# unum-cloud/usearch

Measured on AMD Instinct MI355X. Metric: QPS at recall@10>=0.95, 10000000x768 f16 cos, batch=10000, higher is better.
Workload: dtype f16

## Files before the change

usearch_amd/csrc/common.hpp:

```cpp
#pragma once
#include <cstddef>
#include <cstdint>

namespace usearch_amd {

enum metric_kind_t : std::uint8_t {
    metric_unknown_k = 0,
    metric_ip_k = 'i',
    metric_cos_k = 'c',
    metric_l2sq_k = 'e',
    metric_hamming_k = 'b',
    metric_pearson_k = 'p',
    metric_haversine_k = 'h',
    metric_divergence_k = 'd',
    metric_jaccard_k = 'j',
    metric_tanimoto_k = 't',
    metric_sorensen_k = 's',
};

enum scalar_kind_t : std::uint8_t {
    scalar_unknown_k = 0,
    scalar_b1x8_k = 1,
    scalar_bf16_k = 4,
    scalar_f64_k = 10,
// ... 46 lines not shown
    std::uint32_t dimensions;
    std::uint32_t m, m0;
    std::uint32_t max_level;
    std::uint32_t entry_slot;
    std::uint32_t has_tombstones;
    const std::uint8_t* sketch;
    const float* sketch_directions;
};

struct search_args_t {
    const std::uint8_t* queries;
    std::uint64_t query_stride;
    const std::uint32_t* todo;
    std::uint32_t count;
    std::uint32_t wanted;
    std::uint32_t ef;
    std::uint64_t* keys;
    float* distances;
    std::uint64_t* counts;
    std::uint64_t* visited;
    std::uint64_t* computed;
    std::uint32_t* status;
    std::uint32_t* queue;
    std::uint32_t* peaks;
    std::uint32_t hash_cap;
    std::uint32_t next_cap;
    std::uint8_t* scratch;
    std::uint64_t scratch_stride;
    const std::uint32_t* query_ids;
    std::uint32_t beam_level;
    std::uint32_t emit_slots;
    std::uint32_t descent_only;
    const std::uint32_t* allow_bits;
    const std::uint32_t* known_bits;
    std::uint32_t* ask_slots;
    std::uint64_t* ask_keys;
    std::uint32_t* ask_cursor;
    std::uint32_t ask_cap;
    std::uint32_t guess_threshold;
    std::uint32_t exclude_own;
    unsigned long long* phases;
    std::uint32_t team_offset;
    unsigned long long* wave_clock;
    std::uint32_t seen_offset;
    std::uint32_t seen_cells;
    std::uint32_t early_rows;
    std::uint32_t probe_mode;
    std::uint32_t claim_offset;
    std::uint32_t claim_bits;
    std::uint32_t aside_offset;
    std::uint32_t aside_cells;
    unsigned long long* sketch_counters;
    std::uint32_t sketch_offset;
};

enum : std::uint32_t { status_done_k = 0, status_overflow_k = 1 };

enum probe_mode_t : std::uint32_t {
    probe_swap_k = 0,
    probe_load_first_k = 1,
    probe_plain_k = 2,
};

}
```

usearch_amd/csrc/engine.hip:

```cpp
#include "engine.hpp"

#include <algorithm>
#include <atomic>
#include <chrono>
#include <cstdio>
#include <cstdlib>
#include <cstring>
#include <thread>

#include <hipcub/hipcub.hpp>

#include "casts.hpp"
#include "host_util.hpp"
#include "kernels.hpp"

namespace usearch_amd {

static constexpr std::uint32_t default_probe_mode_k = probe_swap_k;
static constexpr std::size_t default_early_rows_k = 1;

static hipError_t scratch_malloc(void** out, std::size_t bytes) {
#ifdef USEARCH_AMD_EXPERIMENT_SCRATCH_MEMORY
    const std::size_t kind = env_size("USEARCH_AMD_SCRATCH_MEMORY", 0);
    if (kind == 1 || kind == 2) {
// ... 674 lines not shown
        return "Unknown scratch mode";
    const bool top_in_memory = tuning.top_in_memory || env_size("USEARCH_AMD_TOP_IN_MEMORY", 0) != 0;
    const bool two_cells = lanes_ <= 2 && ef <= 128 && !env_size("USEARCH_AMD_NO_TWO_CELLS", 0);
    const std::uint32_t entries_per_lane = top_in_memory ? 0u : ef <= 64 ? 1u : two_cells ? 2u : ef <= 256 ? 4u : ef <= 512 ? 8u : ef <= 1024 ? 16u : 0u;
    call.entries_per_lane = entries_per_lane;

    const std::uint32_t frontier_request = tuning.frontier ? tuning.frontier : (std::uint32_t)env_size("USEARCH_AMD_FRONTIER", 0);
    const bool filtered = view_.has_tombstones || (extras && (extras->allow_bits || extras->exclude_own));
    const bool in_top_possible = frontier_in_top_capable(scalar_) && entries_per_lane && !filtered && mode_request != 3 &&
                                 view_.size < 0x80000000ull && !(extras && (extras->reference_frontier || extras->descent_only));
    if (frontier_request == 2 && !in_top_possible)
        return "The frontier cannot ride in `top` for this search (integer-valued pair, filter, tombstones or expansion > 1024)";
    const int frontier = (frontier_request == 1 || !in_top_possible) ? frontier_heap_k : frontier_top_k;
    if (frontier == frontier_top_k)
        next_cap = 0;

    const std::uint32_t chunks_per_lane = view_.chunks / lanes_;
    std::uint32_t variant_request = tuning.variant ? tuning.variant : (std::uint32_t)env_size("USEARCH_AMD_VARIANT", 0);
    int variant = variant_u4_w4_k;
    const bool every_build = lanes_ == 8 && all_kernel_builds(kernel_metric(metric_), scalar_);
    if (every_build && chunks_per_lane >= 8) {
        variant = chunks_per_lane >= 12 ? variant_u12_w2_k : variant_u8_w3_k;
        if (frontier == frontier_top_k && chunks_per_lane >= 12)
            variant = count >= 40000 ? variant_u4_w4_k : variant_u12x2_w2_k;
    }
    if (variant_request && variant_request - 1 < (std::uint32_t)variant_count_k && every_build) {
        const int requested = (int)variant_request - 1;
        if (requested == variant_u12x2_w2_k && frontier != frontier_top_k)
            return "That kernel build exists for the in-`top` frontier only";
        variant = requested;
    }
    const bool team = every_build && chunks_per_lane >= 8 && !variant_request && mode_request != 3 &&
                      count <= 2ull * compute_units_ && !(extras && extras->descent_only) && !env_size("USEARCH_AMD_NO_TEAM", 0) &&
                      !tuning.waves_per_cu;
    if (team)
        variant = variant_u12_w2_k;
    call.plain_possible = !team && !view_.has_tombstones && view_.m0 <= 64 && view_.nbr0 &&
                          !(extras && (extras->query_ids || extras->beam_level || extras->descent_only || extras->allow_bits || extras->exclude_own)) &&
                          (lanes_ == 1 ? view_.nbr0_rows != nullptr && view_.chunks == 1 : lanes_ == 2) &&
                          plain_build_exists(kernel_metric(metric_), scalar_, (int)lanes_, variant == variant_u4_w4_k, true, (int)entries_per_lane,
                                             frontier == frontier_heap_k) &&
                          !env_size("USEARCH_AMD_NO_PLAIN", 0);
    const std::uint32_t variant_waves_per_cu =
        4u * (std::uint32_t)kernel_waves(variant, (int)entries_per_lane, frontier, (int)lanes_, call.plain_possible);
    const std::uint32_t waves_cap = tuning.waves_per_cu ? tuning.waves_per_cu
                                                        : (std::uint32_t)env_size("USEARCH_AMD_WAVES_PER_CU", 32);
    call.waves_cap = std::min(waves_cap, variant_waves_per_cu);

    if (tuning.sketch > 2)
        return "Unknown sketch mode";
    const bool sketch_use = view_.sketch && tuning.sketch != 1 && !team && mode_request != 3 &&
                            (variant == variant_u12_w2_k || variant == variant_u12x2_w2_k) &&
                            !(extras && (extras->query_ids || extras->beam_level || extras->descent_only || extras->reference_frontier));
    const std::uint32_t sketch_lds = sketch_use ? sketch_columns_k * 4 + 16 : 0;
    auto lds_bytes_for = [&](int mode, std::uint32_t cap_next, std::uint32_t cap_hash) -> std::uint64_t {
        if (mode == scratch_global_k)
            return query_lds;
        const scratch_layout_t l = scratch_layout(entries_per_lane ? 0 : ef, cap_next,
                                                  mode == scratch_lds_k ? (std::uint64_t)cap_hash * 4 : 0);
        return query_lds + l.total + sketch_lds;
    };
    auto waves_for = [&](std::uint64_t lds_bytes) -> std::uint32_t {
        const std::uint64_t granule = (lds_bytes + lds_granule_k - 1) / lds_granule_k * lds_granule_k;
        return (std::uint32_t)std::max<std::uint64_t>(
            1, std::min<std::uint64_t>(call.waves_cap, lds_budget / std::max<std::uint64_t>(granule, 1)));
    };
    const bool default_next_cap = !tuning.next_cap && !env_size("USEARCH_AMD_NEXT_CAP", 0);
    if (default_next_cap && next_cap && mode_request != 1 && mode_request != 3) {
        const std::uint32_t now = waves_for(lds_bytes_for(scratch_hash_k, next_cap, hash_cap));
        if (now < call.waves_cap) {
            const std::uint64_t room = lds_budget / (now + 1) / lds_granule_k * lds_granule_k;
            const std::uint64_t fixed = lds_bytes_for(scratch_hash_k, 0, hash_cap);
            if (room > fixed) {
                const std::uint32_t trimmed = (std::uint32_t)((room - fixed) / 8 / 2 * 2);
                if (trimmed < next_cap && trimmed + 128 >= next_cap)
                    next_cap = trimmed;
            }
        }
    }
    std::uint64_t lds_mode_bytes = lds_bytes_for(scratch_lds_k, next_cap, hash_cap);
    if (!tuning.hash_cap && !env_size("USEARCH_AMD_HASH_CAP", 0) && mode_request == 0 && lds_mode_bytes > lds_budget) {
        const std::uint32_t tighter = std::min<std::uint32_t>(
            pow2_ceil(std::max<std::uint32_t>(1024, (ef * 30 + 1600) / 3 * 4)),
            pow2_ceil((std::uint32_t)std::min<std::uint64_t>(view_.size * 2 + 128, 1u << 30)));
        const std::uint64_t tighter_bytes = lds_bytes_for(scratch_lds_k, next_cap, tighter);
        if (tighter < hash_cap && tighter_bytes <= lds_budget && count <= (std::uint64_t)waves_for(tighter_bytes) * compute_units_ &&
            !env_size("USEARCH_AMD_NO_SMALL_BATCH_LDS", 0)) {
            hash_cap = tighter;
            lds_mode_bytes = tighter_bytes;
        }
    }
    const bool small_batch = lds_mode_bytes <= lds_budget && count <= (std::uint64_t)waves_for(lds_mode_bytes) * compute_units_ &&
                             !env_size("USEARCH_AMD_NO_SMALL_BATCH_LDS", 0);
    int mode = mode_request == 1 ? scratch_lds_k : mode_request == 2 ? scratch_hash_k : mode_request == 3 ? scratch_global_k
               : (small_batch || waves_for(lds_mode_bytes) >= std::min<std::uint32_t>(8, call.waves_cap) ? scratch_lds_k : scratch_hash_k);
    call.mode = mode;
    call.hash_cap = hash_cap;
    call.next_cap = next_cap;

    if (const char* e = ws.reserve(count, 0))
        return e;

    search_args_t& args = call.args;
    args = search_args_t{};
    args.queries = static_cast<const std::uint8_t*>(queries);
    args.query_stride = stride_bytes;
    args.wanted = (std::uint32_t)wanted;
// ... 134 lines not shown
            }
            args.aside_offset = 0, args.aside_cells = 0;
            const bool plain_wanted = call.plain_possible && !args.query_ids && !args.beam_level && !args.descent_only && !args.allow_bits &&
                                      !args.exclude_own && args.probe_mode == probe_swap_k && (lanes_ == 1 || args.early_rows != 0);
#ifdef USEARCH_AMD_EXPERIMENT_NO_ASIDE
            const bool aside_wanted = false;
#else
            const bool aside_wanted = plain_wanted && lanes_ == 2;
#endif
            if (aside_wanted) {
                std::uint32_t aside_cells = 512;
                if (const std::size_t forced_cells = env_size("USEARCH_AMD_ASIDE_CELLS", 0))
                    for (aside_cells = 64; aside_cells * 2 <= forced_cells && aside_cells < 2048; aside_cells *= 2) {}
                const std::uint64_t expected_visits = std::min<std::uint64_t>((std::uint64_t)call.ef * 20 + 800, view_.size);
                const bool room = expected_visits * expected_visits / (2ull * call.hash_cap) <= aside_cells * 3ull / 4 ||
                                  env_size("USEARCH_AMD_PLAIN_WHATEVER_THE_ROOM", 0);
                const std::uint64_t with_aside = (wave_lds_bytes + 15) / 16 * 16 + aside_cells * 4ull;
                if (room && waves_for(with_aside) >= waves_for(wave_lds_bytes) && with_aside <= lds_budget) {
                    args.aside_offset = (std::uint32_t)((wave_lds_bytes + 15) / 16 * 16);
                    args.aside_cells = aside_cells;
                    wave_lds_bytes = with_aside;
                }
            }
            const std::size_t forced = env_size("USEARCH_AMD_SEEN_CELLS", (std::size_t)-1);
            std::uint32_t cells = 0;
            if (forced != (std::size_t)-1) {
                for (cells = 1; cells * 2 <= forced && cells < 8192; cells *= 2) {}
                cells = forced ? cells : 0;
            } else {
                for (std::uint32_t candidate = 2048; candidate >= 128 && !cells; candidate /= 2)
                    if (waves_for((wave_lds_bytes + 15) / 16 * 16 + candidate * 4ull) >= waves_for(wave_lds_bytes))
                        cells = candidate;
            }
            if (cells && (wave_lds_bytes + 15) / 16 * 16 + cells * 4ull <= lds_budget) {
                args.seen_offset = (std::uint32_t)((wave_lds_bytes + 15) / 16 * 16);
                args.seen_cells = cells;
                wave_lds_bytes = args.seen_offset + cells * 4ull;
            }
            call.stats.probe_mode = args.probe_mode;
            call.stats.seen_cells = args.seen_cells;
            call.stats.claim_bits = args.claim_bits;
        }
        params.plain = 0;
        if (call.mode == scratch_hash_k && !params.team && lanes_ <= 2 && call.plain_possible && !args.query_ids && !args.beam_level &&
            !args.descent_only && !args.allow_bits && !args.exclude_own && args.probe_mode == probe_swap_k && (lanes_ == 1 || args.early_rows != 0)) {
#ifdef USEARCH_AMD_EXPERIMENT_NO_ASIDE
            params.plain = args.seen_cells ? 1u : 0u;
#else
            params.plain = (lanes_ == 2 ? args.aside_cells : args.seen_cells) ? 1u : 0u;
#endif
        }
        call.stats.plain = params.plain;
        call.stats.aside_cells = args.aside_cells;
        args.sketch_offset = 0;
        if (args.sketch_counters) {
            const std::uint64_t offset = (wave_lds_bytes + 15) / 16 * 16;
            if (!params.team && offset + sketch_columns_k * 4 <= lds_budget) {
                args.sketch_offset = (std::uint32_t)offset;
                wave_lds_bytes = offset + sketch_columns_k * 4;
            } else {
                args.sketch_counters = nullptr;
            }
        }
        const std::uint64_t lds_bytes = params.team ? (wave_lds_bytes + 15) / 16 * 16 + team_bytes : wave_lds_bytes;
        args.team_offset = params.team ? (std::uint32_t)((wave_lds_bytes + 15) / 16 * 16) : 0u;
        const std::uint32_t grid = params.team ? pending
                                               : (std::uint32_t)std::min<std::uint64_t>(pending, (std::uint64_t)waves_for(lds_bytes) * compute_units_);
        const std::uint64_t slab = call.mode == scratch_hash_k ? (std::uint64_t)call.hash_cap * 4 : 0;
        const std::size_t scratch_draws = std::min<std::size_t>(8, env_size("USEARCH_AMD_SCRATCH_DRAWS", 8));
        const bool draw_scratch = slab * grid > ws.scratch_bytes && slab * grid >= ((std::uint64_t)8 << 20) && scratch_draws > 1 &&
                                  pending >= 2ull * grid && grid >= 2u * (std::uint32_t)compute_units_ &&
                                  !env_size("USEARCH_AMD_SCRATCH_REDRAW", 0);
        if (const char* e = ws.reserve(call.count, draw_scratch ? 0 : slab * grid))
            return e;
        args.status = ws.d_status, args.peaks = ws.d_peaks;
        args.hash_cap = call.hash_cap;
        args.next_cap = call.next_cap;
        args.todo = call.have_todo ? ws.d_todo : nullptr;
        args.count = pending;
        args.scratch = ws.d_scratch;
        args.scratch_stride = slab;
        args.wave_clock = nullptr;
        if (draw_scratch) {
            params.mode = call.mode;
            params.entries_per_lane = call.entries_per_lane;
            params.grid = grid;
            params.lds_bytes = (std::uint32_t)lds_bytes;
            hipEvent_t begin = nullptr, end = nullptr;
            UA_HIP(hipEventCreate(&begin));
            if (hipError_t created = hipEventCreate(&end); created != hipSuccess) {
                (void)hipEventDestroy(begin);
                return hip_message(created);
            }
            void* candidates[8] = {nullptr};
            float trial_ms[8] = {0};
            std::size_t drawn = 0;
            const char* failure = nullptr;
            auto trial = [&](void* block, float& ms) -> const char* {
                args.scratch = static_cast<std::uint8_t*>(block);
                args.count = grid;
                for (int repeat = 0; repeat < 2; ++repeat) {
                    hipError_t e = hipMemsetAsync(ws.d_queue, 0, 8, stream);
                    if (e == hipSuccess)
                        e = hipEventRecord(begin, stream);
                    if (e == hipSuccess)
                        e = launch_search(metric_, scalar_, params, view_, args);
                    if (e == hipSuccess)
                        e = hipEventRecord(end, stream);
                    if (e == hipSuccess)
                        e = hipEventSynchronize(end);
                    if (e == hipSuccess)
                        e = hipEventElapsedTime(&ms, begin, end);
// ... 182 lines not shown
            std::memcpy(counters, ws.h_status + 2, 16);
            call.stats.sketch_tested += counters[0], call.stats.sketch_pruned += counters[1];
        }
        if (call.params.mode == scratch_global_k) {
            if (ws.h_status[1])
                return "Search scratch overflow in the global-memory pass";
            break;
        }
        if (!ws.h_status[1])
            break;
        UA_HIP(hipMemcpyAsync(ws.h_status + 16, ws.d_status, call.count * 4, hipMemcpyDeviceToHost, stream));
        UA_HIP(hipStreamSynchronize(stream));
        std::vector<std::uint32_t> again;
        if (call.have_todo) {
            for (std::uint32_t q : call.todo)
                if (ws.h_status[16 + q] == status_overflow_k)
                    again.push_back(q);
        } else {
            for (std::uint32_t q = 0; q < call.count; ++q)
                if (ws.h_status[16 + q] == status_overflow_k)
                    again.push_back(q);
        }
        call.todo.swap(again);
        call.have_todo = true;
        call.reran = true;
        if (call.todo.empty())
            break;
        if (rung == 0) {
            call.stats.retried_lds = (std::uint32_t)call.todo.size();
            call.mode = scratch_hash_k;
            call.hash_cap = std::min<std::uint32_t>(call.hash_cap * 4, pow2_ceil((std::uint32_t)std::min<std::uint64_t>(view_.size * 2 + 128, 1u << 30)));
            if (call.next_cap) {
                const std::uint32_t lds_budget = (std::uint32_t)env_size("USEARCH_AMD_LDS_BUDGET", 160 * 1024);
                call.next_cap = (std::uint32_t)std::min<std::uint64_t>((std::uint64_t)call.next_cap * 4, view_.size + 64);
                while (call.next_cap > 64 &&
                       call.query_lds + scratch_layout(call.entries_per_lane ? 0 : call.ef, call.next_cap, 0).total > lds_budget)
                    call.next_cap = call.next_cap * 3 / 4;
            }
        } else {
            call.mode = scratch_global_k;
        }
        if (call.mode != scratch_global_k)
            UA_HIP(hipMemcpyAsync(ws.d_todo, call.todo.data(), call.todo.size() * 4, hipMemcpyHostToDevice, stream));
        if (const char* e = run_ladder(call))
            return e;
    }

    if (call.want_phases) {
        unsigned long long ticks[16] = {0};
        UA_HIP(hipMemcpy(ticks, call.args.phases, 128, hipMemcpyDeviceToHost));
        double total = 0;
        for (int i = 0; i < 6; ++i)
            total += (double)ticks[i];
        std::fprintf(stderr, "[usearch_amd] phases ef=%u grid=%u: setup %.1f%% pop+list %.1f%% visited %.1f%% distances %.1f%% "
                             "commit %.1f%% [heap push %.1f%% top insert %.1f%%, %llu candidates rechecked] dump %.1f%% (%.3g ticks); "
                             "frontier pushes %llu, lists ready ahead %llu\n",
                     call.ef, first_grid, 100 * ticks[0] / total, 100 * ticks[1] / total, 100 * ticks[2] / total,
                     100 * ticks[3] / total, 100 * ticks[4] / total, 100 * ticks[8] / total, 100 * ticks[9] / total, ticks[10],
                     100 * ticks[5] / total, total, ticks[6], ticks[7]);
        if (ticks[15])
            std::fprintf(stderr, "[usearch_amd] a team's helpers: %llu hops, ticks measuring per hop %.0f %.0f %.0f %.0f\n", ticks[15],
                         (double)ticks[11] / (double)ticks[15], (double)ticks[12] / (double)ticks[15],
                         (double)ticks[13] / (double)ticks[15], (double)ticks[14] / (double)ticks[15]);
    }
    if (call.want_clock && ws.d_wave_clock && first_grid) {
        std::vector<unsigned long long> clock((std::size_t)first_grid * 2);
        UA_HIP(hipMemcpy(clock.data(), ws.d_wave_clock, clock.size() * 8, hipMemcpyDeviceToHost));
        unsigned long long first = ~0ull, last = 0;
        for (std::uint32_t w = 0; w < first_grid; ++w)
            first = std::min(first, clock[2 * w]), last = std::max(last, clock[2 * w + 1]);
        double gone = 0;
        for (std::uint32_t w = 0; w < first_grid; ++w)
            gone += (double)(clock[2 * w] - first) + (double)(last - clock[2 * w + 1]);
        const double span = (double)(last - first);
        call.stats.tail_idle = span > 0 ? (float)(gone / (span * first_grid)) : 0.f;
        call.stats.span_ms = (float)(span / 1e5);
        if (env_size("USEARCH_AMD_WAVE_CLOCK", 0) > 1) {
            unsigned long long bins[10] = {0};
            for (std::uint32_t w = 0; w < first_grid; ++w)
                ++bins[std::min<std::size_t>(9, (std::size_t)(10.0 * (double)(clock[2 * w + 1] - first) / std::max(span, 1.0)))];
            std::fprintf(stderr, "[usearch_amd] wave exits by tenth of the %.3f ms span (grid %u):", call.stats.span_ms, first_grid);
            for (unsigned long long b : bins)
                std::fprintf(stderr, " %llu", b);
            std::fprintf(stderr, "; idle share %.4f\n", call.stats.tail_idle);
        }
    }
    call.stats.passes = call.passes;
    call.stats.kernel_ms = call.total_ms;
    call.stats.mode = (std::uint32_t)first_mode + 1;
    call.stats.grid = first_grid;
    call.stats.lds_bytes = first_lds;
    if (stats)
        *stats = call.stats;
    if (call.sketch_auto && call.count >= 1024)
        judge_sketch(call.stats.sketch_tested, call.stats.sketch_pruned);
    return nullptr;
}

const char* snapshot_t::search_device(const void* queries, std::size_t count, std::size_t stride_bytes,
                                      std::size_t wanted, std::size_t expansion, std::uint64_t* keys,
                                      float* distances, std::uint64_t* counts, std::uint64_t* visited,
                                      std::uint64_t* computed, hipStream_t stream, const search_tuning_t& tuning,
                                      search_stats_t* stats, bool timed, const search_extras_t* extras) {
    if (stats)
        *stats = search_stats_t{};
    search_call_t call;
    const char* error = search_begin(call, queries, count, stride_bytes, wanted, expansion, keys, distances, counts, visited,
                                     computed, stream, tuning, timed, extras);
    if (error) {
        if (call.workspace)
            give_back(call.workspace);
        return error;
// ... 466 lines not shown
```

usearch_amd/csrc/kernels.hpp:

```cpp
#pragma once
#include <type_traits>
#include <hip/hip_runtime.h>

#include "common.hpp"
#include "sketch.hpp"

namespace usearch_amd {

#define UA_DEVICE __device__ __forceinline__


UA_DEVICE std::uint32_t lane_id() { return threadIdx.x & 63u; }

template <bool global_ak> UA_DEVICE void wave_sync() {
    if constexpr (global_ak) {
        __builtin_amdgcn_fence(__ATOMIC_RELEASE, "workgroup");
        __builtin_amdgcn_wave_barrier();
        __builtin_amdgcn_fence(__ATOMIC_ACQUIRE, "workgroup");
    } else {
        __builtin_amdgcn_fence(__ATOMIC_RELEASE, "workgroup", "local");
        __builtin_amdgcn_wave_barrier();
        __builtin_amdgcn_fence(__ATOMIC_ACQUIRE, "workgroup", "local");
    }
}
// ... 960 lines not shown
UA_DEVICE void team_touch_rows(const snapshot_view_t& ix, const std::uint32_t* ahead, std::uint32_t helper, team_landing_t& landing) {
    const std::uint32_t lane = lane_id();
    const std::uint32_t row = helper * 8 + (lane >> 3);
    const std::uint32_t slot = row < team_ahead_rows_k ? ahead[row] : none_slot_k;
    const std::uint32_t halves = (ix.bytes_per_vector + 63u) / 64u;
    const std::uint8_t* half = ix.vectors + (std::uint64_t)slot * ix.row_stride + (lane & 7u) * 64u;
    if (slot != none_slot_k && (lane & 7u) < halves)
        asm volatile("global_load_dword %0, %1, off" : "=&v"(landing.cell[0]) : "v"(half) : "memory");
    if (slot != none_slot_k && 8u + (lane & 7u) < halves)
        asm volatile("global_load_dword %0, %1, off" : "=&v"(landing.cell[1]) : "v"(half + 512) : "memory");
    if (slot != none_slot_k && 16u + (lane & 7u) < halves)
        asm volatile("global_load_dword %0, %1, off" : "=&v"(landing.cell[2]) : "v"(half + 1024) : "memory");
}
UA_DEVICE void team_landing_alive(const team_landing_t& landing) {
    asm volatile("" ::"v"(landing.cell[0]), "v"(landing.cell[1]), "v"(landing.cell[2]));
}

constexpr int team_waves_k = 5;

UA_DEVICE void team_barrier() { asm volatile("s_waitcnt lgkmcnt(0)\n\ts_barrier" ::: "memory"); }

template <int metric_ak, int scalar_ak, int lanes_ak, int loads_ak>
UA_DEVICE void team_share(const snapshot_view_t& ix, const std::uint8_t* query_lds, query_norm_t a2, const std::uint32_t* slots,
                          float* out, std::uint32_t count, std::uint32_t part, std::uint32_t parts, bool in_turn = false) {
    const std::uint32_t per_part = in_turn ? 64u / lanes_ak : (count + parts - 1) / parts;
    const std::uint32_t begin = part * per_part;
    const std::uint32_t end = (in_turn && part + 1 == parts) || begin + per_part > count ? count : begin + per_part;
    if (begin < end)
        measure_rows<metric_ak, scalar_ak, lanes_ak, loads_ak, false, 1>(ix, query_lds, a2, slots + begin, out + begin, end - begin);
}

template <int metric_ak, int scalar_ak, int lanes_ak, int unroll_ak, int mode_ak, int epl_ak, int frontier_ak, int team_ak = 1,
          bool plain_ak = false>
UA_DEVICE bool search_one(const snapshot_view_t& ix, const search_args_t& args, std::uint32_t q,
                          std::uint8_t* query_lds, std::uint8_t* heaps, std::uint32_t* visits, team_t* team = nullptr) {
    constexpr bool global_ak = mode_ak == scratch_global_k;
    constexpr bool in_top_ak = frontier_ak == frontier_top_k;
    static_assert(!in_top_ak || (epl_ak > 0 && !global_ak), "the frontier rides in the register layout of `top`");
    static_assert(!plain_ak || (lanes_ak <= 2 && mode_ak == scratch_hash_k && team_ak == 1 && !in_top_ak), "short rows over the global hash");
    using mem = scratch_gt<global_ak>;
    const std::uint32_t lane = lane_id();
    const std::uint32_t ef = args.ef, wanted = args.wanted;
    const scratch_layout_t layout = scratch_layout(epl_ak ? 0 : ef, in_top_ak ? 0 : args.next_cap, 0);
    top_gt<epl_ak, global_ak, in_top_ak> top;
    top.reset(reinterpret_cast<cand_t*>(heaps + layout.top));
    cand_t* next = reinterpret_cast<cand_t*>(heaps + layout.next);
    std::uint32_t* cand_slots = reinterpret_cast<std::uint32_t*>(heaps + layout.cand_slots);
    float* cand_distances = reinterpret_cast<float*>(heaps + layout.cand_distances);
    const std::uint32_t visits_mask = global_ak ? 0u : args.hash_cap - 1;
    const std::uint32_t visits_limit = global_ak ? 0xFFFFFFFFu : args.hash_cap - args.hash_cap / 4;

#ifdef USEARCH_AMD_PHASES
    std::uint64_t phase_mark = args.phases ? __builtin_amdgcn_s_memtime() : 0;
    std::uint64_t phase_ticks[6] = {0, 0, 0, 0, 0, 0};
    std::uint32_t diagnostic_pushes = 0, diagnostic_ready = 0, diagnostic_rechecks = 0;
    std::uint64_t diagnostic_push_ticks = 0, diagnostic_insert_ticks = 0;
    auto tick = [&](int phase) {
        if (args.phases) {
            const std::uint64_t now = __builtin_amdgcn_s_memtime();
            phase_ticks[phase] += now - phase_mark;
            phase_mark = now;
        }
    };
#else
    auto tick = [](int) {};
#endif
    const std::uint64_t query_row = !plain_ak && args.query_ids ? args.query_ids[q] : q;
    const query_norm_t a2 = stage_query<metric_ak, scalar_ak, lanes_ak>(
        ix, args.queries + query_row * args.query_stride, query_lds);

    if constexpr (!global_ak) {
        uint4* cells = reinterpret_cast<uint4*>(visits);
        const uint4 empty = {none_slot_k, none_slot_k, none_slot_k, none_slot_k};
        for (std::uint32_t i = lane; i < args.hash_cap / 4; i += 64)
            cells[i] = empty;
#ifdef USEARCH_AMD_EXPERIMENT_NO_SLAB_CLEAR_WAIT
        wave_sync<false>();
#else
        if constexpr (mode_ak == scratch_hash_k)
            wave_sync<true>();
        else
            wave_sync<false>();
#endif
    }

    constexpr bool seen_ak = lanes_ak <= 2 && mode_ak == scratch_hash_k && team_ak == 1;
#ifdef USEARCH_AMD_EXPERIMENT_NO_ASIDE
    constexpr bool aside_ak = false;
#else
    constexpr bool aside_ak = plain_ak && lanes_ak == 2;
#endif
    std::uint32_t* seen = nullptr;
    std::uint32_t seen_mask = 0;
    std::uint32_t* aside = nullptr;
    std::uint32_t aside_mask = 0, aside_count = 0;
    if constexpr (aside_ak) {
        aside = reinterpret_cast<std::uint32_t*>(query_lds + args.aside_offset);
        aside_mask = args.aside_cells - 1;
        for (std::uint32_t i = lane; i < args.aside_cells; i += 64)
            aside[i] = none_slot_k;
        wave_sync<false>();
    }
    if constexpr (seen_ak) {
        if (args.seen_cells) {
            seen = reinterpret_cast<std::uint32_t*>(query_lds + args.seen_offset);
            seen_mask = args.seen_cells - 1;
            for (std::uint32_t i = lane; i < args.seen_cells; i += 64)
// ... 38 lines not shown
        }
    }

    std::uint32_t computed = 0, cycles = 0;
    constexpr int loads_ak = unroll_ak % 100, rows_ak = unroll_ak / 100 + 1;
    auto measure = [&](std::uint32_t count) {
        measure_rows<metric_ak, scalar_ak, lanes_ak, loads_ak, global_ak, 1>(ix, query_lds, a2, cand_slots, cand_distances,
                                                                            count);
        computed += count;
    };
    auto measure_hop = [&](std::uint32_t count, float radius_now) {
        if constexpr (sketch_ak) {
            if (sketch_on && top.size == ef) {
                const std::uint32_t sub = lane & 7u, group = lane >> 3;
                const float* coefficients = reinterpret_cast<const float*>(query_lds + args.sketch_offset) + sub * 8;
                const float4 q0 = *reinterpret_cast<const float4*>(coefficients), q1 = *reinterpret_cast<const float4*>(coefficients + 4);
                const std::uint32_t my_slot = lane < count ? mem::load(cand_slots + lane) : 0u;
                for (std::uint32_t base = 0; base < count; base += 32) {
                    uint4 record[4];
#pragma unroll
                    for (int r = 0; r < 4; ++r) {
                        const std::uint32_t ci = base + (std::uint32_t)r * 8 + group;
                        record[r] = uint4{0u, 0u, 0u, 0u};
                        if (ci < count)
                            record[r] = *reinterpret_cast<const uint4*>(ix.sketch + (std::uint64_t)mem::load(cand_slots + ci) * sketch_record_bytes_k + sub * 16);
                    }
#pragma unroll
                    for (int r = 0; r < 4; ++r) {
                        const std::uint32_t ci = base + (std::uint32_t)r * 8 + group;
                        const uint4 v = record[r];
                        const std::uint32_t last = sub == 7u ? 0u : v.w;
                        float dot = 0.f;
                        dot = __builtin_fmaf(half_bits_to_float(v.x & 0xFFFFu), q0.x, dot);
                        dot = __builtin_fmaf(half_bits_to_float(v.x >> 16), q0.y, dot);
                        dot = __builtin_fmaf(half_bits_to_float(v.y & 0xFFFFu), q0.z, dot);
                        dot = __builtin_fmaf(half_bits_to_float(v.y >> 16), q0.w, dot);
                        dot = __builtin_fmaf(half_bits_to_float(v.z & 0xFFFFu), q1.x, dot);
                        dot = __builtin_fmaf(half_bits_to_float(v.z >> 16), q1.y, dot);
                        dot = __builtin_fmaf(half_bits_to_float(last & 0xFFFFu), q1.z, dot);
                        dot = __builtin_fmaf(half_bits_to_float(last >> 16), q1.w, dot);
                        float residual = sub == 7u ? __builtin_bit_cast(float, v.w) : 0.f;
#pragma unroll
                        for (int offset = 1; offset < 8; offset <<= 1) {
                            dot += xor_lane(dot, offset);
                            residual += xor_lane(residual, offset);
                        }
                        if (sub == 0u && ci < count)
                            mem::store(cand_distances + ci, sketch_lower_bound(dot, residual, sketch_margin));
                    }
                }
                wave_sync<false>();
                const float bound = lane < count ? mem::load(cand_distances + lane) : 0.f;
                const std::uint64_t survivors = ballot(lane < count && !(bound >= radius_now));
                const std::uint32_t kept = popcount64(survivors);
                sketch_tested += count, sketch_pruned += count - kept;
                if (kept < count) {
                    const bool survivor = lane_bit(survivors);
                    const std::uint32_t rank = rank_below(survivors, lane);
                    wave_sync<false>();
                    if (survivor)
                        mem::store(cand_slots + rank, my_slot);
                    wave_sync<false>();
                    if (kept)
                        measure_rows<metric_ak, scalar_ak, lanes_ak, loads_ak, global_ak, rows_ak>(ix, query_lds, a2, cand_slots, cand_distances, kept);
                    const float mine = survivor ? mem::load(cand_distances + rank) : bound;
                    wave_sync<false>();
                    if (lane < count) {
                        mem::store(cand_slots + lane, my_slot);
                        mem::store(cand_distances + lane, mine);
                    }
                    wave_sync<false>();
                    computed += count;
                    return;
                }
            }
        }
        if constexpr (team_ak > 1) {
            if (lane == 0)
                team->count = count, team->leader_in = 1u, team->a2 = a2;
            team_barrier();
            team_share<metric_ak, scalar_ak, lanes_ak, loads_ak>(ix, query_lds, a2, cand_slots, cand_distances, count, 0, 4);
            team_barrier();
        } else {
            measure_rows<metric_ak, scalar_ak, lanes_ak, loads_ak, global_ak, rows_ak>(ix, query_lds, a2, cand_slots,
                                                                                       cand_distances, count);
        }
        computed += count;
    };
    auto allowed = [&](std::uint32_t slot) -> bool {
        if constexpr (plain_ak)
            return true;
        if (!ix.has_tombstones && !args.allow_bits && !args.exclude_own)
            return true;
        bool ok = !(args.exclude_own && slot == (std::uint32_t)query_row);
        if (ok && ix.has_tombstones)
            ok = ix.keys[slot] != free_key_k;
        if (ok && args.allow_bits) {
            const std::uint32_t word = slot >> 5, bit = 1u << (slot & 31);
            if (args.known_bits && !(args.known_bits[word] & bit)) {
                ok = slot * 0x9E3779B1u <= args.guess_threshold;
                if (lane == 0) {
                    const std::uint32_t at = atomicAdd(args.ask_cursor, 1u);
                    if (at < args.ask_cap)
                        args.ask_slots[at] = slot, args.ask_keys[at] = ix.keys[slot];
                }
            } else {
// ... 257 lines not shown
        if (!list_ready && lane < cells)
            first_cell = list[lane];
        uint4 inline_row = {0u, 0u, 0u, 0u};
        if constexpr (inline_ak) {
            if (inline_rows) {
                if (list_ready)
                    inline_row = ahead_row;
                else if (lane < cells)
                    inline_row = reinterpret_cast<const uint4*>(ix.nbr0_rows)[(std::uint64_t)expanded * cells + lane];
            }
        }
        bool popped = false;
        auto pop_now = [&]() {
            popped = true;
            ahead_slot = none_slot_k;
            if constexpr (in_top_ak) {
                float ahead_distance;
                std::uint32_t ahead_lane, ahead_index;
                if (!top.first_open(ahead_distance, ahead_slot, ahead_lane, ahead_index))
                    ahead_slot = none_slot_k;
            } else {
                heap_pop<global_ak>(next, next_size);
                if (next_size)
                    ahead_slot = uniform_u32(cand_slot(mem::load(next)));
            }
            if (ahead_slot != none_slot_k) {
                ahead_cell = lane < cells ? list_of(ahead_slot)[lane] : none_slot_k;
                if constexpr (inline_ak)
                    if (inline_rows && lane < cells)
                        ahead_row = reinterpret_cast<const uint4*>(ix.nbr0_rows)[(std::uint64_t)ahead_slot * cells + lane];
            }
        };
        if (in_top_ak || !list_ready || cells > 64 || mode_ak == scratch_global_k)
            pop_now();
        for (std::uint32_t tile = 0; tile < cells; tile += 64) {
            const std::uint32_t cell = tile + lane;
            const std::uint32_t neighbor =
                tile == 0 ? (list_ready ? ready_cell : first_cell) : (cell < cells ? list[cell] : none_slot_k);
            const bool present = neighbor != none_slot_k;
            const std::uint32_t present_count = popcount64(ballot(present));
            if (!present_count)
                break;
            if (visits_count + present_count > visits_limit ||
                (!in_top_ak && next_size - (popped ? 0u : 1u) + present_count > args.next_cap)) {
                overflow = true;
                break;
            }
            tick(1);
            bool fresh;
            float early_mine = 0.f;
            bool early_done = false;
            std::uint64_t asked_mask = 0;
            bool measured_early = false;
            if constexpr (mode_ak == scratch_global_k) {
                fresh = visits_set<mode_ak>(visits, visits_mask, neighbor, present);
            } else {
                std::uint32_t h = hash_slot(neighbor) & visits_mask;
                std::uint32_t old = neighbor;
                bool asks = present;
                std::uint32_t seen_cell = 0;
                if constexpr (seen_ak) {
                    if (seen) {
                        seen_cell = ((neighbor * 0x9E3779B1u) >> 9) & seen_mask;
                        asks = present && seen[seen_cell] != neighbor;
                    }
                }
                bool shadow_done = false;
                auto shadow_work = [&]() {
                    if (shadow_done)
                        return;
                    shadow_done = true;
                if constexpr (inline_ak) {
                    if (inline_rows) {
                        partial_t p;
                        accumulate_chunk<metric_ak, scalar_ak>(p, query_lds, 0, inline_row);
                        early_mine = finalize_distance<metric_ak, scalar_ak>(p, a2, ix.dimensions);
                        early_done = true;
                    }
                }
                if constexpr (early_ak) {
                    if (early_rows && tile == 0) {
                        asked_mask = ballot(asks);
                        const std::uint32_t asked = popcount64(asked_mask);
                        if (asks)
                            cand_slots[rank_below(asked_mask, lane)] = neighbor;
                        wave_sync<false>();
                        if (asked)
                            measure_rows<metric_ak, scalar_ak, lanes_ak, loads_ak, false, 1>(ix, query_lds, a2, cand_slots, cand_distances, asked);
                        measured_early = true;
                    }
                }
                };
                std::uint32_t probe_mode = probe_swap_k;
#ifdef USEARCH_AMD_EXPERIMENT_PROBE_MODES
                if constexpr (seen_ak)
                    probe_mode = args.probe_mode;
#endif
                const bool load_first = probe_mode == probe_load_first_k;
                if (probe_mode == probe_plain_k) {
                    std::uint32_t* claim = reinterpret_cast<std::uint32_t*>(query_lds + args.claim_offset);
                    const std::uint32_t claim_mask = args.claim_bits - 1;
                    bool looking = asks;
                    for (;;) {
                        std::uint32_t cell_value = none_slot_k;
                        if (looking)
                            cell_value = __hip_atomic_load(visits + h, __ATOMIC_RELAXED, __HIP_MEMORY_SCOPE_AGENT);
                        if (!popped)
                            pop_now();
                        shadow_work();
                        const bool wants = looking && cell_value == none_slot_k;
                        if (looking && cell_value == neighbor)
                            looking = false;
                        if (ballot(wants)) {
                            const std::uint32_t bit = h & claim_mask;
                            bool won = false;
                            if (wants) {
                                const std::uint32_t before = __hip_atomic_fetch_or(claim + (bit >> 5), 1u << (bit & 31u), __ATOMIC_RELAXED,
                                                                                   __HIP_MEMORY_SCOPE_WORKGROUP);
                                won = ((before >> (bit & 31u)) & 1u) == 0u;
                                claim[bit >> 5] = 0u;
                            }
                            if (won) {
                                __hip_atomic_store(visits + h, neighbor, __ATOMIC_RELAXED, __HIP_MEMORY_SCOPE_AGENT);
                                old = none_slot_k, looking = false;
                            }
                        }
                        if (looking && !wants)
                            h = (h + 1) & visits_mask;
                        if (!ballot(looking))
                            break;
                    }
                } else {
                if (asks) {
                    if (load_first) {
                        old = __hip_atomic_load(visits + h, __ATOMIC_RELAXED, __HIP_MEMORY_SCOPE_AGENT);
                        if (old == none_slot_k)
                            old = atomicCAS(visits + h, none_slot_k, neighbor);
                    } else {
                        old = atomicCAS(visits + h, none_slot_k, neighbor);
                    }
                }
                if (!popped)
                    pop_now();
                shadow_work();
                if constexpr (aside_ak) {
                    bool taken = asks && old != none_slot_k && old != neighbor;
                    const std::uint64_t taken_mask = ballot(taken);
                    if (taken_mask) {
                        if (aside_count + popcount64(taken_mask) > aside_mask - aside_mask / 4) {
                            overflow = true;
                            break;
                        }
                        std::uint32_t cell = ((neighbor * 0x9E3779B1u) >> 11) & aside_mask;
                        do {
                            std::uint32_t there = neighbor;
                            if (taken)
                                there = atomicCAS(aside + cell, none_slot_k, neighbor);
                            if (taken && (there == none_slot_k || there == neighbor))
                                old = there, taken = false;
                            cell = (cell + 1) & aside_mask;
                        } while (ballot(taken));
                        aside_count += popcount64(ballot(lane_bit(taken_mask) && old == none_slot_k));
                    }
                }
                while (!aside_ak && old != none_slot_k && old != neighbor) {
                    h = (h + 1) & visits_mask;
                    if (load_first) {
                        old = __hip_atomic_load(visits + h, __ATOMIC_RELAXED, __HIP_MEMORY_SCOPE_AGENT);
                        if (old == none_slot_k)
                            old = atomicCAS(visits + h, none_slot_k, neighbor);
                    } else {
                        old = atomicCAS(visits + h, none_slot_k, neighbor);
                    }
                }
                }
                fresh = present && old == none_slot_k;
                if constexpr (seen_ak) {
                    if (seen && asks)
                        seen[seen_cell] = neighbor;
                }
            }
            const std::uint64_t fresh_mask = ballot(fresh);
            tick(2);
            const std::uint32_t count = popcount64(fresh_mask);
            visits_count += count;
            if (!count)
                continue;
            float mine = 0.f;
            std::uint32_t mine_slot = 0u;
            bool candidate;
            if (inline_rows) {
                if constexpr (inline_ak) {
                    if (early_done) {
                        mine = early_mine;
                    } else {
                        partial_t p;
                        accumulate_chunk<metric_ak, scalar_ak>(p, query_lds, 0, inline_row);
                        mine = finalize_distance<metric_ak, scalar_ak>(p, a2, ix.dimensions);
                    }
                }
                mine_slot = neighbor;
                candidate = fresh;
                computed += count;
            } else if (measured_early) {
                mine = fresh ? cand_distances[rank_below(asked_mask, lane)] : 0.f;
                mine_slot = neighbor;
                candidate = fresh;
                computed += count;
                wave_sync<false>();
            } else {
                if (fresh)
                    mem::store(cand_slots + rank_below(fresh_mask, lane), neighbor);
                wave_sync<global_ak>();
                measure_hop(count, radius);
                mine = lane < count ? mem::load(cand_distances + lane) : 0.f;
                mine_slot = lane < count ? mem::load(cand_slots + lane) : 0u;
                candidate = lane < count;
            }
            tick(3);

            std::uint64_t pending = ballot(candidate && (top.size < ef || mine < radius));
            while (pending) {
                const std::uint32_t i = (std::uint32_t)__ffsll((long long)pending) - 1;
                pending &= pending - 1;
                const float d = read_lane_f32(mine, i);
#ifdef USEARCH_AMD_PHASES
                ++diagnostic_rechecks;
#endif
                if (!(top.size < ef || d < radius))
                    continue;
                const std::uint32_t successor = read_lane_u32(mine_slot, i);
#ifdef USEARCH_AMD_PHASES
                ++diagnostic_pushes;
                const std::uint64_t t0 = __builtin_amdgcn_s_memtime();
#endif
                push_ticket_t ticket;
                if constexpr (!in_top_ak)
                    ticket = heap_push_begin<global_ak>(next, next_size);
#ifdef USEARCH_AMD_PHASES
                const std::uint64_t t1 = __builtin_amdgcn_s_memtime();
#endif
                if (in_top_ak || allowed(successor))
                    top.insert(d, successor, ef, radius);
                if constexpr (!in_top_ak)
                    heap_push_finish<global_ak>(next, next_size, ticket, -d, successor);
#ifdef USEARCH_AMD_PHASES
                const std::uint64_t t2 = __builtin_amdgcn_s_memtime();
                diagnostic_push_ticks += t1 - t0, diagnostic_insert_ticks += t2 - t1;
#endif
            }
            peak_next = next_size > peak_next ? next_size : peak_next;
            wave_sync<global_ak>();
            tick(4);
        }
        if (overflow)
            break;
        if (!popped)
            pop_now();
    }

    if (overflow) {
        if (lane == 0) {
            args.status[q] = status_overflow_k;
            atomicAdd(args.queue + 1, 1u);
        }
        return false;
    }
    const std::uint32_t found = top.size < wanted ? top.size : wanted;
    top.dump(ix, args, q, found, wanted);
    tick(5);
#ifdef USEARCH_AMD_PHASES
    if (args.phases && lane == 0) {
#pragma unroll
        for (int phase = 0; phase < 6; ++phase)
            atomicAdd(args.phases + phase, (unsigned long long)phase_ticks[phase]);
        atomicAdd(args.phases + 6, (unsigned long long)diagnostic_pushes);
        atomicAdd(args.phases + 7, (unsigned long long)diagnostic_ready);
        atomicAdd(args.phases + 8, (unsigned long long)diagnostic_push_ticks);
        atomicAdd(args.phases + 9, (unsigned long long)diagnostic_insert_ticks);
        atomicAdd(args.phases + 10, (unsigned long long)diagnostic_rechecks);
    }
#endif
    if constexpr (sketch_ak) {
        if (sketch_tested && lane == 0) {
            atomicAdd(args.sketch_counters, (unsigned long long)sketch_tested);
            atomicAdd(args.sketch_counters + 1, (unsigned long long)sketch_pruned);
        }
    }
    if (lane == 0) {
        args.counts[q] = found;
        args.visited[q] = cycles;
        args.computed[q] = computed;
        args.status[q] = status_done_k;
        if (args.peaks) {
            args.peaks[2 * (std::uint64_t)q] = peak_next;
            args.peaks[2 * (std::uint64_t)q + 1] = visits_count;
        }
    }
    return true;
}

enum kernel_variant_t : int {
    variant_u4_w4_k = 0,
    variant_u8_w3_k = 1,
    variant_u12_w2_k = 2,
    variant_u12x2_w2_k = 3,
    variant_count_k = 4,
};
#ifndef USEARCH_AMD_TINY_ROW_WAVES
#define USEARCH_AMD_TINY_ROW_WAVES 6
#endif
#ifndef USEARCH_AMD_SHORT_ROW_WAVES
#define USEARCH_AMD_SHORT_ROW_WAVES 5
#endif
#ifndef USEARCH_AMD_PLAIN_TINY_ROW_WAVES
#define USEARCH_AMD_PLAIN_TINY_ROW_WAVES USEARCH_AMD_TINY_ROW_WAVES
#endif
constexpr int variant_unroll(int v) { return v == variant_u4_w4_k ? 4 : v == variant_u8_w3_k ? 8 : 12; }
constexpr int variant_rows(int v) { return v == variant_u12x2_w2_k ? 2 : 1; }
constexpr int kernel_waves(int variant, int epl, int frontier = 0, int lanes = 8, bool plain = false) {
    if (variant == variant_u12x2_w2_k)
        return 2;
    if (plain && variant == variant_u4_w4_k && epl == 1 && lanes == 1)
        return USEARCH_AMD_PLAIN_TINY_ROW_WAVES;
    if (variant == variant_u4_w4_k && epl == 1 && lanes <= 2)
        return lanes == 1 ? USEARCH_AMD_TINY_ROW_WAVES : USEARCH_AMD_SHORT_ROW_WAVES;
    if (variant == variant_u4_w4_k && epl == 2 && lanes <= 2)
        return USEARCH_AMD_SHORT_ROW_WAVES;
// ... 210 lines not shown
```

usearch_amd/csrc/sketch.hpp:

```cpp
#pragma once
#include <cmath>
#include <cstdint>
#include <cstring>
#include <vector>

#include "common.hpp"

#ifndef __HIPCC__
#define USEARCH_AMD_SKETCH_BOTH inline
#else
#define USEARCH_AMD_SKETCH_BOTH __host__ __device__ inline
#endif

namespace usearch_amd {

constexpr std::uint32_t sketch_rank_k = 62;
constexpr std::uint32_t sketch_columns_k = 64;
constexpr std::uint32_t sketch_record_bytes_k = 128;
constexpr std::uint32_t sketch_min_row_bytes_k = 1536;
constexpr std::uint64_t sketch_seed_k = 0x5EEDC0DE5EEDC0DEull;

inline bool sketch_eligible(metric_kind_t metric, scalar_kind_t scalar, std::size_t bytes_per_row) {
    return metric == metric_cos_k && (scalar == scalar_f32_k || scalar == scalar_f16_k || scalar == scalar_bf16_k) &&
           bytes_per_row >= sketch_min_row_bytes_k;
}

USEARCH_AMD_SKETCH_BOTH bool sketch_norm_in_range(double n2) { return n2 >= 0x1p-100 && n2 <= 0x1p100; }

USEARCH_AMD_SKETCH_BOTH float sketch_slack(std::uint32_t dimensions) { return 16.f * (float)dimensions * 0x1p-24f + 0x1p-16f; }

USEARCH_AMD_SKETCH_BOTH float sketch_residual(double s1, double s2, double gram_defect) {
    double r2 = 1.0 - 2.0 * s1 + (1.0 + gram_defect) * s2 + 1e-9;
    r2 = r2 > 0.0 ? r2 : 0.0;
    return (float)sqrt(r2) * 1.000001f + 1e-30f;
}

USEARCH_AMD_SKETCH_BOTH float sketch_lower_bound(float dot, float residual, float slack) { return 1.f - ((dot + residual) + slack); }

USEARCH_AMD_SKETCH_BOTH float sketch_scalar(const std::uint8_t* row, std::uint32_t i, scalar_kind_t scalar) {
    if (scalar == scalar_f32_k) {
        float v;
        memcpy(&v, row + 4 * (std::size_t)i, 4);
        return v;
    }
    std::uint16_t bits;
    memcpy(&bits, row + 2 * (std::size_t)i, 2);
    if (scalar == scalar_bf16_k) {
        const std::uint32_t wide = (std::uint32_t)bits << 16;
        float v;
        memcpy(&v, &wide, 4);
        return v;
    }
    _Float16 h;
    memcpy(&h, &bits, 2);
    return (float)h;
}

struct sketch_directions_t {
    std::vector<float> transposed;
    std::uint32_t rank = 0;
    double gram_defect = 0.0;
};

inline std::uint64_t sketch_sample_slot(std::uint64_t k, std::uint64_t size) {
    std::uint64_t z = sketch_seed_k + (k + 1) * 0x9E3779B97F4A7C15ull;
    z = (z ^ (z >> 30)) * 0xBF58476D1CE4E5B9ull;
    z = (z ^ (z >> 27)) * 0x94D049BB133111EBull;
    z ^= z >> 31;
    return size ? z % size : 0;
}

// ... 142 lines not shown
```

Before: 363,200.

## Prefetch neighbor sketch records into LDS during visited-set work and bound early

When the top list is full on the first tile, the kernel issues asynchronous global-to-LDS loads of every neighbor's 128-byte sketch record while the visited-set probing runs. It then computes the sketch lower bounds from LDS, prunes candidates whose bound exceeds the radius, and measures full rows only for the survivors. The aim is to hide sketch-record latency behind the hash work rather than fetching records after the candidate list is built. In exchange it spends extra LDS per wave, which can reduce occupancy, fetches records for neighbors that turn out to be already visited, and adds a vmcnt(0) wait. Phase-timing diagnostics for the sketch are also added.

```diff
diff --git a/usearch_amd/csrc/common.hpp b/usearch_amd/csrc/common.hpp
--- a/usearch_amd/csrc/common.hpp
+++ b/usearch_amd/csrc/common.hpp
@@ -122,6 +122,7 @@
     std::uint32_t aside_cells;
     unsigned long long* sketch_counters;
     std::uint32_t sketch_offset;
+    std::uint32_t sketch_records_offset;
 };
 
 enum : std::uint32_t { status_done_k = 0, status_overflow_k = 1 };
diff --git a/usearch_amd/csrc/engine.hip b/usearch_amd/csrc/engine.hip
--- a/usearch_amd/csrc/engine.hip
+++ b/usearch_amd/csrc/engine.hip
@@ -750,7 +750,7 @@
     const bool sketch_use = view_.sketch && tuning.sketch != 1 && !team && mode_request != 3 &&
                             (variant == variant_u12_w2_k || variant == variant_u12x2_w2_k) &&
                             !(extras && (extras->query_ids || extras->beam_level || extras->descent_only || extras->reference_frontier));
-    const std::uint32_t sketch_lds = sketch_use ? sketch_columns_k * 4 + 16 : 0;
+    const std::uint32_t sketch_lds = sketch_use ? sketch_columns_k * 4 + 16 + sketch_records_lds_bytes(view_.m0) : 0;
     auto lds_bytes_for = [&](int mode, std::uint32_t cap_next, std::uint32_t cap_hash) -> std::uint64_t {
         if (mode == scratch_global_k)
             return query_lds;
@@ -991,12 +991,16 @@
         }
         call.stats.plain = params.plain;
         call.stats.aside_cells = args.aside_cells;
-        args.sketch_offset = 0;
+        args.sketch_offset = 0, args.sketch_records_offset = 0;
         if (args.sketch_counters) {
             const std::uint64_t offset = (wave_lds_bytes + 15) / 16 * 16;
             if (!params.team && offset + sketch_columns_k * 4 <= lds_budget) {
                 args.sketch_offset = (std::uint32_t)offset;
                 wave_lds_bytes = offset + sketch_columns_k * 4;
+                if (wave_lds_bytes + sketch_records_lds_bytes(view_.m0) <= lds_budget && !env_size("USEARCH_AMD_NO_SKETCH_SHADOW", 0)) {
+                    args.sketch_records_offset = (std::uint32_t)wave_lds_bytes;
+                    wave_lds_bytes += sketch_records_lds_bytes(view_.m0);
+                }
             } else {
                 args.sketch_counters = nullptr;
             }
@@ -1285,12 +1289,18 @@
         double total = 0;
         for (int i = 0; i < 6; ++i)
             total += (double)ticks[i];
+        const bool sketch_phase = !ticks[15] && ticks[11];
+        if (sketch_phase)
+            total += (double)ticks[11];
         std::fprintf(stderr, "[usearch_amd] phases ef=%u grid=%u: setup %.1f%% pop+list %.1f%% visited %.1f%% distances %.1f%% "
                              "commit %.1f%% [heap push %.1f%% top insert %.1f%%, %llu candidates rechecked] dump %.1f%% (%.3g ticks); "
                              "frontier pushes %llu, lists ready ahead %llu\n",
                      call.ef, first_grid, 100 * ticks[0] / total, 100 * ticks[1] / total, 100 * ticks[2] / total,
                      100 * ticks[3] / total, 100 * ticks[4] / total, 100 * ticks[8] / total, 100 * ticks[9] / total, ticks[10],
                      100 * ticks[5] / total, total, ticks[6], ticks[7]);
+        if (sketch_phase)
+            std::fprintf(stderr, "[usearch_amd] phases ef=%u, the sketch: records and bounds %.1f%%, survivors' rows %.1f%% (\"distances\" above)\n",
+                         call.ef, 100 * ticks[11] / total, 100 * ticks[3] / total);
         if (ticks[15])
             std::fprintf(stderr, "[usearch_amd] a team's helpers: %llu hops, ticks measuring per hop %.0f %.0f %.0f %.0f\n", ticks[15],
                          (double)ticks[11] / (double)ticks[15], (double)ticks[12] / (double)ticks[15],
diff --git a/usearch_amd/csrc/kernels.hpp b/usearch_amd/csrc/kernels.hpp
--- a/usearch_amd/csrc/kernels.hpp
+++ b/usearch_amd/csrc/kernels.hpp
@@ -1036,7 +1036,7 @@
 
 #ifdef USEARCH_AMD_PHASES
     std::uint64_t phase_mark = args.phases ? __builtin_amdgcn_s_memtime() : 0;
-    std::uint64_t phase_ticks[6] = {0, 0, 0, 0, 0, 0};
+    std::uint64_t phase_ticks[7] = {0, 0, 0, 0, 0, 0, 0};
     std::uint32_t diagnostic_pushes = 0, diagnostic_ready = 0, diagnostic_rechecks = 0;
     std::uint64_t diagnostic_push_ticks = 0, diagnostic_insert_ticks = 0;
     auto tick = [&](int phase) {
@@ -1181,6 +1181,7 @@
                 wave_sync<false>();
                 const float bound = lane < count ? mem::load(cand_distances + lane) : 0.f;
                 const std::uint64_t survivors = ballot(lane < count && !(bound >= radius_now));
+                tick(6);
                 const std::uint32_t kept = popcount64(survivors);
                 sketch_tested += count, sketch_pruned += count - kept;
                 if (kept < count) {
@@ -1544,6 +1545,9 @@
             bool early_done = false;
             std::uint64_t asked_mask = 0;
             bool measured_early = false;
+            bool records_early = false;
+            if constexpr (sketch_ak)
+                records_early = tile == 0 && sketch_on && top.size == ef && args.sketch_records_offset != 0u;
             if constexpr (mode_ak == scratch_global_k) {
                 fresh = visits_set<mode_ak>(visits, visits_mask, neighbor, present);
             } else {
@@ -1634,6 +1638,20 @@
                 }
                 if (!popped)
                     pop_now();
+                if constexpr (sketch_ak) {
+                    if (records_early) {
+                        std::uint8_t* records = query_lds + args.sketch_records_offset;
+                        const std::uint32_t tile_cells = cells < 64u ? cells : 64u;
+#pragma nounroll
+                        for (std::uint32_t r = 0; r * 8 < tile_cells; ++r) {
+                            const std::uint32_t listed = (std::uint32_t)__builtin_amdgcn_ds_bpermute((int)((r * 8 + (lane >> 3)) << 2), (int)neighbor);
+                            const std::uint32_t member = listed == none_slot_k ? 0u : listed;
+                            __builtin_amdgcn_global_load_lds(
+                                (const __attribute__((address_space(1))) void*)(ix.sketch + (std::uint64_t)member * sketch_record_bytes_k + (lane & 7u) * 16u),
+                                (__attribute__((address_space(3))) void*)(records + r * 1024u), 16, 0, 0);
+                        }
+                    }
+                }
                 shadow_work();
                 if constexpr (aside_ak) {
                     bool taken = asks && old != none_slot_k && old != neighbor;
@@ -1673,6 +1691,8 @@
                 }
             }
             const std::uint64_t fresh_mask = ballot(fresh);
+            if (records_early)
+                asm volatile("s_waitcnt vmcnt(0)" ::: "memory");
             tick(2);
             const std::uint32_t count = popcount64(fresh_mask);
             visits_count += count;
@@ -1700,6 +1720,56 @@
                 candidate = fresh;
                 computed += count;
                 wave_sync<false>();
+            } else if (records_early) {
+                mine_slot = neighbor;
+                candidate = fresh;
+                if constexpr (sketch_ak) {
+                    const std::uint8_t* records = query_lds + args.sketch_records_offset;
+                    const std::uint32_t sub = lane & 7u, group = lane >> 3;
+                    const float* coefficients = reinterpret_cast<const float*>(query_lds + args.sketch_offset) + sub * 8;
+                    const float4 q0 = *reinterpret_cast<const float4*>(coefficients), q1 = *reinterpret_cast<const float4*>(coefficients + 4);
+#pragma nounroll
+                    for (std::uint32_t r = 0; r < 8; ++r) {
+                        if (!((fresh_mask >> (r * 8)) & 0xFFu))
+                            continue;
+                        const std::uint32_t position = r * 8 + group;
+                        const uint4 v = *reinterpret_cast<const uint4*>(records + position * sketch_record_bytes_k + sub * 16);
+                        const std::uint32_t last = sub == 7u ? 0u : v.w;
+                        float dot = 0.f;
+                        dot = __builtin_fmaf(half_bits_to_float(v.x & 0xFFFFu), q0.x, dot);
+                        dot = __builtin_fmaf(half_bits_to_float(v.x >> 16), q0.y, dot);
+                        dot = __builtin_fmaf(half_bits_to_float(v.y & 0xFFFFu), q0.z, dot);
+                        dot = __builtin_fmaf(half_bits_to_float(v.y >> 16), q0.w, dot);
+                        dot = __builtin_fmaf(half_bits_to_float(v.z & 0xFFFFu), q1.x, dot);
+                        dot = __builtin_fmaf(half_bits_to_float(v.z >> 16), q1.y, dot);
+                        dot = __builtin_fmaf(half_bits_to_float(last & 0xFFFFu), q1.z, dot);
+                        dot = __builtin_fmaf(half_bits_to_float(last >> 16), q1.w, dot);
+                        float residual = sub == 7u ? __builtin_bit_cast(float, v.w) : 0.f;
+#pragma unroll
+                        for (int offset = 1; offset < 8; offset <<= 1) {
+                            dot += xor_lane(dot, offset);
+                            residual += xor_lane(residual, offset);
+                        }
+                        if (sub == 0u)
+                            mem::store(cand_distances + position, sketch_lower_bound(dot, residual, sketch_margin));
+                    }
+                    wave_sync<false>();
+                    const float bound = fresh ? mem::load(cand_distances + lane) : 0.f;
+                    const std::uint64_t survivors = ballot(fresh && !(bound >= radius));
+                    const std::uint32_t kept = popcount64(survivors);
+                    sketch_tested += count, sketch_pruned += count - kept;
+                    tick(6);
+                    const bool survivor = lane_bit(survivors);
+                    const std::uint32_t rank = rank_below(survivors, lane);
+                    if (survivor)
+                        mem::store(cand_slots + rank, neighbor);
+                    wave_sync<false>();
+                    if (kept)
+                        measure_rows<metric_ak, scalar_ak, lanes_ak, loads_ak, global_ak, rows_ak>(ix, query_lds, a2, cand_slots, cand_distances, kept);
+                    mine = survivor ? mem::load(cand_distances + rank) : bound;
+                    computed += count;
+                    wave_sync<false>();
+                }
             } else {
                 if (fresh)
                     mem::store(cand_slots + rank_below(fresh_mask, lane), neighbor);
@@ -1766,6 +1836,8 @@
 #pragma unroll
         for (int phase = 0; phase < 6; ++phase)
             atomicAdd(args.phases + phase, (unsigned long long)phase_ticks[phase]);
+        if (phase_ticks[6])
+            atomicAdd(args.phases + 11, (unsigned long long)phase_ticks[6]);
         atomicAdd(args.phases + 6, (unsigned long long)diagnostic_pushes);
         atomicAdd(args.phases + 7, (unsigned long long)diagnostic_ready);
         atomicAdd(args.phases + 8, (unsigned long long)diagnostic_push_ticks);
diff --git a/usearch_amd/csrc/sketch.hpp b/usearch_amd/csrc/sketch.hpp
--- a/usearch_amd/csrc/sketch.hpp
+++ b/usearch_amd/csrc/sketch.hpp
@@ -17,6 +17,9 @@
 constexpr std::uint32_t sketch_rank_k = 62;
 constexpr std::uint32_t sketch_columns_k = 64;
 constexpr std::uint32_t sketch_record_bytes_k = 128;
+USEARCH_AMD_SKETCH_BOTH std::uint32_t sketch_records_lds_bytes(std::uint32_t cells) {
+    return ((cells < 64u ? cells : 64u) + 7u) / 8u * 8u * sketch_record_bytes_k;
+}
 constexpr std::uint32_t sketch_min_row_bytes_k = 1536;
 constexpr std::uint64_t sketch_seed_k = 0x5EEDC0DE5EEDC0DEull;
 
```

Result: faster. 371,100 (median of 6 runs) (+2.2%).
